# Tanveer81/ReVisionLLM

Measured on AMD Instinct MI355X. Metric: video-segments/sec (whole node), stage-2 100-seg recursion, Vicuna-7B, higher is better.
Workload: dtype fp16

## Files before the change

revisionllm_amd/build.py:

```python
import os
import subprocess
import sys
from concurrent.futures import ThreadPoolExecutor

HERE = os.path.dirname(os.path.abspath(__file__))
CSRC = os.path.join(HERE, "csrc")
OBJ = os.path.join(CSRC, "build")
FLAVOURS = {"f16": ("librevision_hip.so", "-DRV_OP_F16=1"), "bf16": ("librevision_hip_bf16.so", "-DRV_OP_F16=0")}
LIB = os.path.join(HERE, FLAVOURS["f16"][0])


def lib_path(flavour):
    return os.path.join(HERE, FLAVOURS[flavour][0])
SOURCES = ["error.hip", "init.hip", "gemm.hip", "gemm_pp.hip", "gemm_arows.hip", "gemm_rows.hip", "gemm_rows_p1.hip", "gemm_rows_p2.hip", "gemm_rows_p3.hip", "rowops.hip", "attention.hip", "sample.hip", "similarity.hip", "propose.hip", "prefilter.hip", "frames.hip", "frames_yuv.hip", "engine.hip"]
HEADERS = ["exports.map", "common.h", "kernels.h", "gemv_finish.h", "frames_common.h", "gemm_rows.hip", os.path.join("..", "..", "include", "revision_hip.h")]
FLAGS = ["--offload-arch=gfx950", "-O3", "-std=c++17", "-fPIC", "-fvisibility=hidden", "-fvisibility-inlines-hidden", "-Wall", "-Wno-unused-function",
         "-Wno-pass-failed"]


def _hipcc():
    for c in (os.environ.get("HIPCC"), "/opt/rocm/bin/hipcc", "hipcc"):
        if c and (os.path.isabs(c) and os.path.exists(c) or not os.path.isabs(c)):
            return c
    raise RuntimeError("hipcc not found")


def _stale(target, deps):
    if not os.path.exists(target):
        return True
    t = os.path.getmtime(target)
    return any(os.path.getmtime(d) > t for d in deps)


def build_library(force=False, verbose=False, flavours=("f16", "bf16")):
    hipcc = _hipcc()
    hdrs = [os.path.join(CSRC, h) for h in HEADERS]
    jobs = []
    for fl in flavours:
        os.makedirs(os.path.join(OBJ, fl), exist_ok=True)
        for s in SOURCES:
            src = os.path.join(CSRC, s)
            obj = os.path.join(OBJ, fl, s.replace(".hip", ".o"))
            if force or _stale(obj, [src] + hdrs):
                jobs.append([hipcc] + FLAGS + [FLAVOURS[fl][1], "-DRV_TU=" + s.replace(".hip", ""), "-c", src, "-o", obj])

    def run(cmd):
        r = subprocess.run(cmd, capture_output=True, text=True)
        if r.returncode != 0:
            raise RuntimeError("hipcc failed: %s\n%s" % (" ".join(cmd), r.stderr))
        if verbose and r.stderr:
            sys.stderr.write(r.stderr)

    with ThreadPoolExecutor(max_workers=int(os.environ.get("REVISION_BUILD_JOBS", "7"))) as ex:
        list(ex.map(run, jobs))
    for fl in flavours:
        objs = [os.path.join(OBJ, fl, s.replace(".hip", ".o")) for s in SOURCES]
        lib = lib_path(fl)
        if force or _stale(lib, objs):
            run([hipcc, "--offload-arch=gfx950", "-shared", "-fPIC", "-Wl,--version-script=" + os.path.join(CSRC, "exports.map"), "-o", lib] + objs)
    return LIB


if __name__ == "__main__":
    fl = tuple(a for a in sys.argv[1:] if a in FLAVOURS) or tuple(FLAVOURS)
    print(build_library(force="--force" in sys.argv, verbose=True, flavours=fl))
```

revisionllm_amd/csrc/gemm_rows.hip:

```cpp
#include <hip/hip_runtime.h>

#include <atomic>
#include <type_traits>

#include "kernels.h"
#include "gemv_finish.h"

#ifndef RS_PROBE
#define RS_PROBE 0
#endif
#ifndef RS_PART
#define RS_PART 0
#endif
#ifndef RS_DW_BIG
#define RS_DW_BIG 4
#endif

namespace {

typedef const __attribute__((address_space(1))) void* gptr_t;
typedef __attribute__((address_space(3))) void* lptr_t;
__device__ __forceinline__ void glds16(const void* g, void* l) { __builtin_amdgcn_global_load_lds((gptr_t)g, (lptr_t)l, 16, 0, 0); }

typedef unsigned int rs_u32x4 __attribute__((ext_vector_type(4)));
constexpr int RS_SC1 = 16;
__device__ __forceinline__ void st_sc1(__amdgpu_buffer_rsrc_t r, unsigned byte_off, f32x4 v) {
    __builtin_amdgcn_raw_buffer_store_b128(__builtin_bit_cast(rs_u32x4, v), r, (int)byte_off, 0, RS_SC1);
}
__device__ __forceinline__ f32x4 ld_sc1(__amdgpu_buffer_rsrc_t r, unsigned byte_off) {
    return __builtin_bit_cast(f32x4, __builtin_amdgcn_raw_buffer_load_b128(r, (int)byte_off, 0, RS_SC1));
}

constexpr int RS_W = 4;
constexpr int RS_THREADS = (RS_W + 1) * 64;
template <int MB, int WP = 1> struct RowsCfg {
    static constexpr int DW = WP == 2 ? 8 : (MB >= 8 ? RS_DW_BIG : 4), LPS = WP == 2 ? 2 : 4, DX = MB == 4 ? 4 : 3, WPE = MB <= 5 ? 3 : 2;
};
typedef unsigned int rs_w8 __attribute__((ext_vector_type(4)));

constexpr bool rows_sumsq_at_head(int MB) { return MB >= 8; }
template <int MB, int NTH, int PTB>
__device__ __forceinline__ void rows_sumsq(const GemvNorm& nrm, float* ssq, int tg) {
    if (!nrm.in_sumsq || (RS_PROBE & 16)) return;
    constexpr int CHAINS = MB * 128;
    constexpr int PT = (CHAINS + NTH - 1) / NTH;
    const int nblk = nrm.in_nblk;
    const int off = (RS_PROBE & 2048) ? 0 : (int)((blockIdx.x >> 3) * 37u) % CHAINS;
#pragma unroll
    for (int i0 = 0; i0 < PT; i0 += PTB) {
        f32x4 pj[PTB][8];
        int cc[PTB];
#pragma unroll
        for (int i = 0; i < PTB; ++i) {
            const int idx = tg + (i0 + i) * NTH;
            int c = idx + off;
            c = c >= CHAINS ? c - CHAINS : c;
            cc[i] = (i0 + i < PT && idx < CHAINS) ? c : -1;
            const int mb = c >> 7, q = (c >> 2) & 31, rq = c & 3;
            const float* src = nrm.in_sumsq + ((int64_t)(mb * nblk + q) * 16 + rq * 4);
#pragma unroll
            for (int j = 0; j < 8; ++j) {
                const bool have = q + 32 * j < nblk;
                const f32x4 v = *(const f32x4*)(src + (have ? j * 512 : 0));
                pj[i][j] = have ? v : f32x4{0.f, 0.f, 0.f, 0.f};
            }
        }
        __builtin_amdgcn_sched_barrier(0);
#pragma unroll
        for (int i = 0; i < PTB; ++i) {
            if (cc[i] < 0) continue;
            const int c = cc[i], mb = c >> 7, q = (c >> 2) & 31, rq = c & 3;
            f32x4 a = f32x4{0.f, 0.f, 0.f, 0.f};
#pragma unroll
            for (int j = 0; j < 8; ++j) a += pj[i][j];
            for (int b = q + 256; b < nblk; b += 32) a += *(const f32x4*)(nrm.in_sumsq + ((int64_t)(mb * nblk + b) * 16 + rq * 4));
            *(f32x4*)(ssq + mb * 512 + q * 16 + rq * 4) = a;
        }
    }
}

template <int MB>
__device__ __forceinline__ void rows_sumsq_total(const float* ssq, float* totl, int t) {
    if (t < MB * 16) {
        const int mb = t >> 4, row = t & 15;
        float tot = 0.f;
#pragma unroll
        for (int q = 0; q < 32; ++q) tot += ssq[(mb * 32 + q) * 16 + row];
        totl[t] = tot;
    }
}

template <int MB, int PPW, int PAIRS, int WP>
__device__ __forceinline__ void rows_qkv_finish(const f32x4 (&sres)[PPW], int wave, int cg, int fr, int kg, int M, const GemvNorm& nrm, const QkvRope& qr,
                                                const float* totl) {
    const int D = qr.H * 128;
    const int n0 = cg * 64;
    const int sec = n0 >= 2 * D ? 2 : n0 >= D ? 1 : 0;
    const int hd0 = n0 - sec * D, head = hd0 >> 7;
    int posv[PPW];
    f32x4 cf[PPW], wsc[PPW];
#pragma unroll
    for (int i = 0; i < PPW; ++i) {
        const int p = wave + RS_W * i < PAIRS ? wave + RS_W * i : PAIRS - 1;
        const int tile = p / MB, mb = p % MB, b = mb * 16 + fr;
        const int pc = (hd0 & 127) + tile * 16 + kg * 4;
        const int bc = b < M ? b : M - 1;
        posv[i] = b < M ? qr.row_pos[bc] : -1;
        cf[i] = sec < 2 ? *(const f32x4*)(qr.cs + ((int64_t)bc * 64 + (pc >> 1)) * 2) : f32x4{0.f, 0.f, 0.f, 0.f};
        if constexpr (WP == 2) wsc[i] = *(const f32x4*)(nrm.w_scale + n0 + tile * 16 + kg * 4);
    }
    __builtin_amdgcn_sched_barrier(0);
#pragma unroll
    for (int i = 0; i < PPW; ++i) {
        const int p = wave + RS_W * i;
        if (p >= PAIRS) break;
        const int tile = p / MB, mb = p % MB, b = mb * 16 + fr;
        const int pc = (hd0 & 127) + tile * 16 + kg * 4;
        f32x4 v = sres[i];
        if constexpr (WP == 2) v *= wsc[i];
        if (nrm.in_sumsq) v *= rsqrtf(__fmaf_rn(totl[mb * 16 + fr], nrm.inv_d, nrm.eps));
        const int pos = posv[i];
        if (pos < 0 || pos >= qr.Smax) continue;
        if (sec < 2) {
            const f32x4 t = cf[i];
            const float a0 = __fmaf_rn(v[0], t[0], -__fmul_rn(v[1], t[1])), b0 = __fmaf_rn(v[1], t[0], __fmul_rn(v[0], t[1]));
            const float a1 = __fmaf_rn(v[2], t[2], -__fmul_rn(v[3], t[3])), b1 = __fmaf_rn(v[3], t[2], __fmul_rn(v[2], t[3]));
            const u32x2 o = pack_op16x4(f32x4{a0, b0, a1, b1});
            if (sec == 0) *(u32x2*)((op16_t*)qr.q16 + (int64_t)b * D + hd0 + tile * 16 + kg * 4) = o;
            else *(u32x2*)((op16_t*)qr.kc + (((int64_t)b * qr.H + head) * qr.Smax + pos) * 128 + pc) = o;
        } else {
            op16_t* dst = (op16_t*)qr.vtc + ((int64_t)b * qr.H + head) * 128 * qr.Smax + rv_vt_index(pc, pos);
#pragma unroll
            for (int r = 0; r < 4; ++r) dst[r * 8] = f32_to_op16(v[r]);
        }
    }
}

#ifndef RS_PF_N
#define RS_PF_N 8
#endif
constexpr int RS_PF = RS_PF_N;
#ifndef RS_EARLY_READS
#define RS_EARLY_READS 0
#endif
constexpr bool rows_early(int MB) { return RS_EARLY_READS && MB >= 8 && !(RS_PROBE & (4 | 4096)); }
template <int MB, int WP>
__device__ __forceinline__ void rows_stage_schedule() {
#ifndef RS_NO_STAGE_SCHEDULE
    if constexpr (MB >= 8 && !(RS_PROBE & 4)) {
        constexpr int R = 4 * MB;
        if constexpr (!rows_early(MB)) __builtin_amdgcn_sched_group_barrier(0x100, RS_PF, 0);
#ifdef RS_EARLY_PIN_VMEM
        else __builtin_amdgcn_sched_group_barrier(0x020, WP == 2 ? 2 : 4, 0);
#endif
#pragma unroll
        for (int i = 0; i < R - RS_PF; ++i) {
            __builtin_amdgcn_sched_group_barrier(0x008, 1, 0);
            __builtin_amdgcn_sched_group_barrier(0x100, 1, 0);
        }
        __builtin_amdgcn_sched_group_barrier(0x008, RS_PF, 0);
    }
#endif
}

template <int MB, int VPW, int FIN, int WP = 1>
__global__ __attribute__((amdgpu_flat_work_group_size(RS_THREADS, RS_THREADS), amdgpu_waves_per_eu(RowsCfg<MB>::WPE, RowsCfg<MB>::WPE))) void
rows_kernel(const op16_t* __restrict__ X, const op16_t* __restrict__ W, float* __restrict__ planes, const float* __restrict__ bias,
            const float* res, int64_t ldr, void* Cv, int64_t ldc, int M, int N, int K, GemvNorm nrm, QkvRope qr) {
    extern __shared__ __attribute__((aligned(16))) char rs_smem[];
    constexpr int S = 8 / VPW, LOG = VPW == 8 ? 3 : VPW == 4 ? 2 : VPW == 2 ? 1 : 0;
    constexpr int DW = RowsCfg<MB, WP>::DW, DX = RowsCfg<MB, WP>::DX, LPS = RowsCfg<MB, WP>::LPS;
    constexpr int SLAB = MB * 4096;
    constexpr int XL = MB * 4;
    static_assert((DX - 2) * XL <= 63 && (DW - 2) * LPS <= 63, "vmcnt is a 6-bit counter");
    const int tid = threadIdx.x, lane = tid & 63;
    const int wave = __builtin_amdgcn_readfirstlane(tid >> 6);
    const int cg = blockIdx.x / S, sp = blockIdx.x % S;
    const int nkb = K >> 7;
    const int ntile = cg * RS_W + (wave < RS_W ? wave : 0);
    auto vcount = [&](int i) -> int { return (nkb - (sp * VPW + i) + 7) >> 3; };
    int T = 0;
#pragma unroll
    for (int i = 0; i < VPW; ++i) T += vcount(i);

    f32x4 acc[MB], stk[LOG ? LOG : 1][MB];
#pragma unroll
    for (int mb = 0; mb < MB; ++mb) acc[mb] = f32x4{0.f, 0.f, 0.f, 0.f};

    if (wave == RS_W) {
        int pi = 0, pc = 0;
        auto next_kb = [&]() -> int {
            int kb = -1;
            if (pi < VPW) {
                kb = sp * VPW + pi + 8 * pc;
                if (++pc == vcount(pi)) { pc = 0; ++pi; }
            }
            return kb;
        };
        auto issue = [&](int g) {
            const int kb = next_kb();
            const op16_t* xs = X + (kb >= 0 ? (int64_t)kb * (MB * 2048) : 0) + lane * 8;
            char* dst = rs_smem + (g % DX) * SLAB;
#pragma unroll
            for (int i = 0; i < XL; ++i) glds16(xs + i * 512, dst + i * 1024);
        };
        if constexpr (!(RS_PROBE & 8))
            for (int d = 0; d < DX - 1; ++d) issue(d);
        if constexpr (rows_sumsq_at_head(MB)) {
            if (nrm.in_sumsq && !(RS_PROBE & 16)) __builtin_amdgcn_s_barrier();
        }
        for (int g = 0; g < T; ++g) {
            asm volatile("s_waitcnt vmcnt(%0)" ::"n"((DX - 2) * XL) : "memory");
            if constexpr (!(RS_PROBE & 2)) __builtin_amdgcn_s_barrier();
            if constexpr (!(RS_PROBE & 8)) issue(g + DX - 1);
        }
        asm volatile("s_waitcnt vmcnt(0)" ::: "memory");
    } else {
        const op16_t* wp = W + (int64_t)ntile * (K >> 5) * (WP == 2 ? 256 : 512) + lane * 8;
        typename std::conditional<WP == 2, rs_w8, op16x8>::type wf[DW][LPS];
        int li = 0, lc = 0;
        int ci = 0, cc = 0;
#define RS_ISSUE_W(slot)                                                                                                             \
    do {                                                                                                                             \
        int kb_ = -1;                                                                                                                \
        if (li < VPW) {                                                                                                              \
            kb_ = sp * VPW + li + 8 * lc;                                                                                            \
            if (++lc == vcount(li)) { lc = 0; ++li; }                                                                                \
        }                                                                                                                            \
        const op16_t* ws_ = kb_ >= 0 ? ((RS_PROBE & 1) ? W + lane * 8 + (kb_ & 1) * 2048 : wp + (int64_t)((RS_PROBE & 8192) ? (kb_ + ((int)blockIdx.x * RS_W + wave) * 5) % nkb : kb_) * (WP == 2 ? 1024 : 2048)) : X + lane * 8; \
        _Pragma("unroll") for (int j_ = 0; j_ < LPS; ++j_)                                                                          \
            wf[slot][j_] = __builtin_nontemporal_load((const typename std::remove_reference<decltype(wf[0][0])>::type*)(ws_ + j_ * 512)); \
    } while (0)
#pragma unroll
        for (int d = 0; d < DW - 1; ++d) RS_ISSUE_W(d);
        if constexpr (rows_sumsq_at_head(MB)) {
            if (nrm.in_sumsq && !(RS_PROBE & 16)) {
                float* ssq_ = (float*)(rs_smem + DX * SLAB);
                rows_sumsq<MB, 256, 3>(nrm, ssq_, tid);
                asm volatile("s_waitcnt lgkmcnt(0)" ::: "memory");
                __builtin_amdgcn_s_barrier();
                rows_sumsq_total<MB>(ssq_, ssq_ + MB * 512, tid);
                asm volatile("s_waitcnt lgkmcnt(0)" ::: "memory");
            }
        }
        unsigned long long* stamps = (unsigned long long*)(rs_smem + DX * SLAB + MB * (2048 + 64));
        const bool stamping = (RS_PROBE & 16384) && S == 1 && wave == 0 && blockIdx.x == 8;
#define RS_STAMP(k_)                                                                       \
    if constexpr (RS_PROBE & 16384) {                                                      \
        if (stamping && g < 64) {                                                          \
            const unsigned long long t_ = __builtin_amdgcn_s_memtime();                    \
            if (lane == 0) stamps[g * 4 + (k_)] = t_;                                      \
        }                                                                                  \
    }
        if constexpr (RS_PROBE & 16384) {
            if (stamping) {
                for (int i = lane; i < 256; i += 64) stamps[i] = 0ull;
            }
        }
        for (int g0 = 0; g0 < T; g0 += DW) {
#pragma unroll
            for (int u = 0; u < DW; ++u) {
                const int g = g0 + u;
                if (g < T) {
                    RS_STAMP(0)
                    asm volatile("s_waitcnt vmcnt(%0)" ::"n"((DW - 2) * LPS) : "memory");
                    RS_STAMP(1)
                    if constexpr (!(RS_PROBE & 2)) __builtin_amdgcn_s_barrier();
                    RS_STAMP(2)
                    op16x8 pre[rows_early(MB) ? RS_PF : 1];
                    if constexpr (rows_early(MB)) {
                        const char* xs0 = rs_smem + (g % DX) * SLAB + lane * 16;
#pragma unroll
                        for (int i = 0; i < RS_PF; ++i) pre[i] = *(const op16x8*)(xs0 + i * 1024);
                    }
                    RS_ISSUE_W((u + DW - 1) % DW);
                    {
                        const char* xs = rs_smem + (g % DX) * SLAB + lane * 16;
#pragma unroll
                        for (int j = 0; j < 4; ++j) {
                            op16x8 wj;
                            if constexpr (WP == 2) wj = fp8x8_to_op16x8(wf[u][j >> 1][(j & 1) * 2], wf[u][j >> 1][(j & 1) * 2 + 1]);
                            else wj = wf[u][j];
#pragma unroll
                            for (int mb = 0; mb < MB; ++mb) {
                                const op16x8 xf = (rows_early(MB) && j * MB + mb < RS_PF) ? pre[(j * MB + mb) % RS_PF]
                                                                                           : *(const op16x8*)(xs + ((RS_PROBE & 4096) ? 0 : (j * MB + mb) * 1024));
                                if constexpr (RS_PROBE & 4) {
                                    if (mb == 0) acc[0][0] += __builtin_bit_cast(f32x4, wj)[j & 3] + __builtin_bit_cast(f32x4, xf)[0];
                                } else {
                                    acc[mb] = rv_mfma16(wj, xf, acc[mb]);
                                }
                            }
                        }
                        rows_stage_schedule<MB, WP>();
                    }
                    RS_STAMP(3)
                    if (++cc == vcount(ci)) {
                        if constexpr (VPW > 1) {
                            bool placed = false;
#pragma unroll
                            for (int b = 0; b < LOG; ++b) {
                                if (placed) continue;
                                if ((ci >> b) & 1) {
#pragma unroll
                                    for (int mb = 0; mb < MB; ++mb) acc[mb] = stk[b][mb] + acc[mb];
                                } else {
#pragma unroll
                                    for (int mb = 0; mb < MB; ++mb) stk[b][mb] = acc[mb];
                                    placed = true;
                                }
                            }
                            if (placed) {
#pragma unroll
                                for (int mb = 0; mb < MB; ++mb) acc[mb] = f32x4{0.f, 0.f, 0.f, 0.f};
                            }
                        }
                        cc = 0;
                        ++ci;
                    }
                }
            }
        }
#undef RS_ISSUE_W
#undef RS_STAMP
        if constexpr (RS_PROBE & 16384) {
            if (stamping) {
                asm volatile("s_waitcnt lgkmcnt(0)" ::: "memory");
                for (int i = lane; i < 256; i += 64) ((unsigned long long*)planes)[i] = stamps[i];
            }
        }
    }
    const unsigned plane = (unsigned)(N >> 4) * MB * 1024;
    const __amdgpu_buffer_rsrc_t pr = __builtin_amdgcn_make_buffer_rsrc(planes, 0, 0x7ffffff0, 0x00020000);
    constexpr int XCH_OFF = MB * 2048 > 16384 ? MB * 2048 : 16384;
    static_assert(XCH_OFF + RS_W * MB * 1024 <= DX * MB * 4096, "the exchange area must fit the slab ring");
    char* xch = rs_smem + XCH_OFF;
    if constexpr (S == 1) {
        asm volatile("s_waitcnt vmcnt(0)" ::: "memory");
        __syncthreads();
        if (wave < RS_W) {
#pragma unroll
            for (int mb = 0; mb < MB; ++mb) *(f32x4*)(xch + ((wave * MB + mb) * 64 + lane) * 16) = acc[mb];
        }
    } else {
        if (wave < RS_W) {
            const unsigned off = sp * plane + ((unsigned)ntile * MB * 64 + lane) * 16;
#pragma unroll
            for (int mb = 0; mb < MB; ++mb) st_sc1(pr, off + mb * 1024, acc[mb]);
        }
        asm volatile("s_waitcnt vmcnt(0)" ::: "memory");
    }
    __syncthreads();
    __shared__ int is_last;
    if constexpr (S > 1) {
        if (tid == 0) {
            unsigned* cnt = (unsigned*)nrm.arrive + (LOG * (RV_ROWS_COUNTERS / 4) + cg);
            is_last = __hip_atomic_fetch_add(cnt, 1u, __ATOMIC_RELAXED, __HIP_MEMORY_SCOPE_AGENT) % S == S - 1;
        }
        __syncthreads();
        if (!is_last) return;
    }
    constexpr int NT = (FIN == 1 || FIN == 2) ? 2 : 1;
    constexpr int OUT_BF16 = (FIN == 1 || FIN == 4) ? 1 : 0;
    constexpr int ACT = FIN == 1 ? RV_ACT_SILU_MUL : RV_ACT_NONE;
    constexpr int ROPE = FIN == 3 ? 1 : 0;
    constexpr int BPG = RS_W / NT;
    constexpr int PAIRS = BPG * MB;
    constexpr int PPW = (PAIRS + RS_W - 1) / RS_W;
    const int fr = lane & 15, kg = lane >> 4;
    const int nblk = N / (16 * NT);
    f32x4 pl[PPW][NT][S];
    if (wave < RS_W) {
#pragma unroll
        for (int i = 0; i < PPW; ++i) {
            const int p = wave + RS_W * i < PAIRS ? wave + RS_W * i : PAIRS - 1;
            const int blk = cg * BPG + p / MB, mb = p % MB;
#pragma unroll
            for (int t = 0; t < NT; ++t) {
                if constexpr (S == 1) {
                    pl[i][t][0] = *(const f32x4*)(xch + (((p / MB * NT + t) * MB + mb) * 64 + lane) * 16);
                } else {
                    const unsigned q = (((unsigned)(blk * NT + t) * MB + mb) * 64 + lane) * 16;
#pragma unroll
                    for (int w = 0; w < S; ++w) pl[i][t][w] = ld_sc1(pr, q + w * plane);
                }
            }
        }
    }
    float* ssq = (float*)(rs_smem + (rows_sumsq_at_head(MB) ? DX * SLAB : 0));
    if constexpr (!rows_sumsq_at_head(MB)) {
        if (nrm.in_sumsq && !(RS_PROBE & 16)) {
            rows_sumsq<MB, RS_THREADS, 2>(nrm, ssq, tid);
            __syncthreads();
            rows_sumsq_total<MB>(ssq, ssq + MB * 512, tid);
            __syncthreads();
        }
    }
    const float* totl = ssq + MB * 512;
    if (wave >= RS_W) return;
    if constexpr (ROPE) {
        if (qr.row_pos && qr.G == 1 && !(RS_PROBE & 64)) {
            f32x4 sv[PPW];
#pragma unroll
            for (int i = 0; i < PPW; ++i) {
                if constexpr (S == 8) sv[i] = gemv_tree8(pl[i][0]);
                else if constexpr (S == 4) sv[i] = (pl[i][0][0] + pl[i][0][1]) + (pl[i][0][2] + pl[i][0][3]);
                else if constexpr (S == 2) sv[i] = pl[i][0][0] + pl[i][0][1];
                else sv[i] = pl[i][0][0];
            }
            rows_qkv_finish<MB, PPW, PAIRS, WP>(sv, wave, cg, fr, kg, M, nrm, qr, totl);
            return;
        }
    }
#pragma unroll
    for (int i = 0; i < PPW; ++i) {
        const int p = wave + RS_W * i;
        if (p >= PAIRS) break;
        const int blk = cg * BPG + p / MB, mb = p % MB;
        f32x4 sres[NT];
#pragma unroll
        for (int t = 0; t < NT; ++t) {
            if constexpr (S == 8) sres[t] = gemv_tree8(pl[i][t]);
            else if constexpr (S == 4) sres[t] = (pl[i][t][0] + pl[i][t][1]) + (pl[i][t][2] + pl[i][t][3]);
            else if constexpr (S == 2) sres[t] = pl[i][t][0] + pl[i][t][1];
            else sres[t] = pl[i][t][0];
        }
        const float tot = nrm.in_sumsq ? totl[mb * 16 + fr] : 0.f;
        const f32x4 z = f32x4{0.f, 0.f, 0.f, 0.f};
        gemv_finish<NT, OUT_BF16, ACT, WP, ROPE>(sres, mb, fr, kg, blk, nblk, M, N, bias, res, ldr, Cv, ldc, nrm, qr, tot, z, z, z, z, false);
    }
}

constexpr int RS_MAXIT = 8;
template <int MB, int VPW, int FIN, int WP = 1>
__global__ __attribute__((amdgpu_flat_work_group_size(RS_THREADS, RS_THREADS), amdgpu_waves_per_eu(RowsCfg<MB>::WPE, RowsCfg<MB>::WPE))) void
rows_kernel_p(const op16_t* __restrict__ X, const op16_t* __restrict__ W, float* __restrict__ planes, const float* __restrict__ bias,
            const float* res, int64_t ldr, void* Cv, int64_t ldc, int M, int N, int K, GemvNorm nrm, QkvRope qr) {
    extern __shared__ __attribute__((aligned(16))) char rs_smem[];
    constexpr int S = 8 / VPW, LOG = VPW == 8 ? 3 : VPW == 4 ? 2 : VPW == 2 ? 1 : 0;
    constexpr int DW = RowsCfg<MB, WP>::DW, DX = RowsCfg<MB, WP>::DX, LPS = RowsCfg<MB, WP>::LPS;
    constexpr int SLAB = MB * 4096;
    constexpr int XL = MB * 4;
    static_assert((DX - 2) * XL <= 63 && (DW - 2) * LPS <= 63, "vmcnt is a 6-bit counter");
    const int tid = threadIdx.x, lane = tid & 63;
    const int wave = __builtin_amdgcn_readfirstlane(tid >> 6);
    const int nitems = (N >> 6) * S, G = (int)gridDim.x;
    const int sp = blockIdx.x % S;
    const int nkb = K >> 7;
    const int n_it = (nitems - (int)blockIdx.x + G - 1) / G;
    auto vcount = [&](int i) -> int { return (nkb - (sp * VPW + i) + 7) >> 3; };
    int T = 0;
#pragma unroll
    for (int i = 0; i < VPW; ++i) T += vcount(i);
    const int Tp = (T + DW - 1) / DW * DW;
    const unsigned plane = (unsigned)(N >> 4) * MB * 1024;
    const __amdgpu_buffer_rsrc_t pr = __builtin_amdgcn_make_buffer_rsrc(planes, 0, 0x7ffffff0, 0x00020000);

    f32x4 acc[MB], stk[LOG ? LOG : 1][MB];
#pragma unroll
    for (int mb = 0; mb < MB; ++mb) acc[mb] = f32x4{0.f, 0.f, 0.f, 0.f};

    if (wave == RS_W) {
        int pi = 0, pc = 0, pp = 0, pn = 0;
        auto issue = [&](int g) {
            int kb = -1;
            if (pn < n_it) {
                if (pp < T) {
                    kb = sp * VPW + pi + 8 * pc;
                    if (++pc == vcount(pi)) { pc = 0; ++pi; }
                }
                if (++pp == Tp) { pp = 0; pi = 0; ++pn; }
            }
            const op16_t* xs = X + (kb >= 0 ? (int64_t)kb * (MB * 2048) : 0) + lane * 8;
            char* dst = rs_smem + (g % DX) * SLAB;
#pragma unroll
            for (int i = 0; i < XL; ++i) glds16(xs + i * 512, dst + i * 1024);
        };
        if constexpr (!(RS_PROBE & 8))
            for (int d = 0; d < DX - 1; ++d) issue(d);
        if constexpr (rows_sumsq_at_head(MB)) {
            if (nrm.in_sumsq && !(RS_PROBE & 16)) __builtin_amdgcn_s_barrier();
        }
        const int TT = n_it * Tp;
        for (int g = 0; g < TT; ++g) {
            asm volatile("s_waitcnt vmcnt(%0)" ::"n"((DX - 2) * XL) : "memory");
            if constexpr (!(RS_PROBE & 2)) __builtin_amdgcn_s_barrier();
            if constexpr (!(RS_PROBE & 8)) issue(g + DX - 1);
        }
    } else {
        const int64_t tile_stride = (int64_t)(K >> 5) * (WP == 2 ? 256 : 512);
        const int64_t item_stride = (int64_t)(G / S) * RS_W * tile_stride;
        const op16_t* wp = W + ((int)blockIdx.x / S * RS_W + wave) * tile_stride + lane * 8;
        typename std::conditional<WP == 2, rs_w8, op16x8>::type wf[DW][LPS];
        int li = 0, lc = 0, lp = 0, ln = 0;
#define RS_ISSUE_W(slot)                                                                                                             \
    do {                                                                                                                             \
        const op16_t* ws_ = X + lane * 8;                                                                                            \
        if (ln < n_it) {                                                                                                             \
            if (lp < T) {                                                                                                            \
                const int kb_ = sp * VPW + li + 8 * lc;                                                                              \
                ws_ = (RS_PROBE & 1) ? W + lane * 8 + (kb_ & 1) * 2048 : wp + (int64_t)((RS_PROBE & 8192) ? (kb_ + ((int)blockIdx.x * RS_W + wave) * 5) % (K >> 7) : kb_) * (WP == 2 ? 1024 : 2048);                 \
                if (++lc == vcount(li)) { lc = 0; ++li; }                                                                            \
            }                                                                                                                        \
            if (++lp == Tp) { lp = 0; li = 0; ++ln; wp += item_stride; }                                                             \
        }                                                                                                                            \
        _Pragma("unroll") for (int j_ = 0; j_ < LPS; ++j_)                                                                          \
            wf[slot][j_] = __builtin_nontemporal_load((const typename std::remove_reference<decltype(wf[0][0])>::type*)(ws_ + j_ * 512)); \
    } while (0)
#pragma unroll
        for (int d = 0; d < DW - 1; ++d) RS_ISSUE_W(d);
        if constexpr (rows_sumsq_at_head(MB)) {
            if (nrm.in_sumsq && !(RS_PROBE & 16)) {
                float* ssq_ = (float*)(rs_smem + DX * SLAB);
                rows_sumsq<MB, 256, 3>(nrm, ssq_, tid);
                asm volatile("s_waitcnt lgkmcnt(0)" ::: "memory");
                __builtin_amdgcn_s_barrier();
                rows_sumsq_total<MB>(ssq_, ssq_ + MB * 512, tid);
                asm volatile("s_waitcnt lgkmcnt(0)" ::: "memory");
            }
        }
        int g = 0;
        for (int n = 0; n < n_it; ++n) {
            int ci = 0, cc = 0;
            for (int s0 = 0; s0 < Tp; s0 += DW) {
#pragma unroll
                for (int u = 0; u < DW; ++u, ++g) {
                    asm volatile("s_waitcnt vmcnt(%0)" ::"n"((DW - 2) * LPS) : "memory");
                    if constexpr (!(RS_PROBE & 2)) __builtin_amdgcn_s_barrier();
                    op16x8 pre[rows_early(MB) ? RS_PF : 1];
                    if constexpr (rows_early(MB)) {
                        const char* xs0 = rs_smem + (g % DX) * SLAB + lane * 16;
#pragma unroll
                        for (int i = 0; i < RS_PF; ++i) pre[i] = *(const op16x8*)(xs0 + i * 1024);
                    }
                    RS_ISSUE_W((u + DW - 1) % DW);
                    if (s0 + u < T) {
                        const char* xs = rs_smem + (g % DX) * SLAB + lane * 16;
#pragma unroll
                        for (int j = 0; j < 4; ++j) {
                            op16x8 wj;
                            if constexpr (WP == 2) wj = fp8x8_to_op16x8(wf[u][j >> 1][(j & 1) * 2], wf[u][j >> 1][(j & 1) * 2 + 1]);
                            else wj = wf[u][j];
#pragma unroll
                            for (int mb = 0; mb < MB; ++mb) {
                                const op16x8 xf = (rows_early(MB) && j * MB + mb < RS_PF) ? pre[(j * MB + mb) % RS_PF]
                                                                                           : *(const op16x8*)(xs + ((RS_PROBE & 4096) ? 0 : (j * MB + mb) * 1024));
                                if constexpr (RS_PROBE & 4) {
                                    if (mb == 0) acc[0][0] += __builtin_bit_cast(f32x4, wj)[j & 3] + __builtin_bit_cast(f32x4, xf)[0];
                                } else {
                                    acc[mb] = rv_mfma16(wj, xf, acc[mb]);
                                }
                            }
                        }
                        rows_stage_schedule<MB, WP>();
                        if (++cc == vcount(ci)) {
                            if constexpr (VPW > 1) {
                                bool placed = false;
#pragma unroll
                                for (int b = 0; b < LOG; ++b) {
                                    if (placed) continue;
                                    if ((ci >> b) & 1) {
#pragma unroll
                                        for (int mb = 0; mb < MB; ++mb) acc[mb] = stk[b][mb] + acc[mb];
                                    } else {
#pragma unroll
                                        for (int mb = 0; mb < MB; ++mb) stk[b][mb] = acc[mb];
                                        placed = true;
                                    }
                                }
                                if (placed) {
#pragma unroll
                                    for (int mb = 0; mb < MB; ++mb) acc[mb] = f32x4{0.f, 0.f, 0.f, 0.f};
                                }
                            }
                            cc = 0;
                            ++ci;
                        }
                    }
                }
            }
            if constexpr (S > 1) {
                const unsigned ntile = (unsigned)(((int)blockIdx.x + n * G) / S * RS_W + wave);
                const unsigned off = sp * plane + (ntile * MB * 64 + lane) * 16;
#pragma unroll
                for (int mb = 0; mb < MB; ++mb) {
                    st_sc1(pr, off + mb * 1024, acc[mb]);
                    acc[mb] = f32x4{0.f, 0.f, 0.f, 0.f};
                }
            }
        }
#undef RS_ISSUE_W
    }
    constexpr int XCH_OFF = MB * 2048 > 16384 ? MB * 2048 : 16384;
    static_assert(XCH_OFF + RS_W * MB * 1024 <= DX * MB * 4096, "the exchange area must fit the slab ring");
    char* xch = rs_smem + XCH_OFF;
    asm volatile("s_waitcnt vmcnt(0)" ::: "memory");
    __syncthreads();
    if constexpr (S == 1) {
        if (wave < RS_W) {
#pragma unroll
            for (int mb = 0; mb < MB; ++mb) *(f32x4*)(xch + ((wave * MB + mb) * 64 + lane) * 16) = acc[mb];
        }
        __syncthreads();
    }
    __shared__ int is_last[RS_MAXIT];
    if constexpr (S > 1) {
        if (tid < n_it) {
            unsigned* cnt = (unsigned*)nrm.arrive + (LOG * (RV_ROWS_COUNTERS / 4) + ((int)blockIdx.x + tid * G) / S);
            is_last[tid] = __hip_atomic_fetch_add(cnt, 1u, __ATOMIC_RELAXED, __HIP_MEMORY_SCOPE_AGENT) % S == S - 1;
        }
        __syncthreads();
        bool any = false;
        for (int n = 0; n < n_it; ++n) any = any || is_last[n];
        if (!any) return;
    }
    constexpr int NT = (FIN == 1 || FIN == 2) ? 2 : 1;
    constexpr int OUT_BF16 = (FIN == 1 || FIN == 4) ? 1 : 0;
    constexpr int ACT = FIN == 1 ? RV_ACT_SILU_MUL : RV_ACT_NONE;
    constexpr int ROPE = FIN == 3 ? 1 : 0;
    constexpr int BPG = RS_W / NT;
    constexpr int PAIRS = BPG * MB;
    constexpr int PPW = (PAIRS + RS_W - 1) / RS_W;
    const int fr = lane & 15, kg = lane >> 4;
    const int nblk = N / (16 * NT);
    float* ssq = (float*)(rs_smem + (rows_sumsq_at_head(MB) ? DX * SLAB : 0));
    if constexpr (!rows_sumsq_at_head(MB)) {
        if (nrm.in_sumsq && !(RS_PROBE & 16)) {
            rows_sumsq<MB, RS_THREADS, 2>(nrm, ssq, tid);
            __syncthreads();
            rows_sumsq_total<MB>(ssq, ssq + MB * 512, tid);
            __syncthreads();
        }
    }
    const float* totl = ssq + MB * 512;
    if (wave >= RS_W) return;
    for (int n = 0; n < n_it; ++n) {
        if constexpr (S > 1) {
            if (!is_last[n]) continue;
        }
        const int cg = ((int)blockIdx.x + n * G) / S;
        f32x4 pl[PPW][NT][S];
        if (wave < RS_W) {
#pragma unroll
            for (int i = 0; i < PPW; ++i) {
                const int p = wave + RS_W * i < PAIRS ? wave + RS_W * i : PAIRS - 1;
                const int blk = cg * BPG + p / MB, mb = p % MB;
#pragma unroll
                for (int t = 0; t < NT; ++t) {
                    if constexpr (S == 1) {
                        pl[i][t][0] = *(const f32x4*)(xch + (((p / MB * NT + t) * MB + mb) * 64 + lane) * 16);
                    } else {
                        const unsigned q = (((unsigned)(blk * NT + t) * MB + mb) * 64 + lane) * 16;
#pragma unroll
                        for (int w = 0; w < S; ++w) pl[i][t][w] = ld_sc1(pr, q + w * plane);
                    }
                }
            }
        }
#pragma unroll
        for (int i = 0; i < PPW; ++i) {
            const int p = wave + RS_W * i;
            if (p >= PAIRS) break;
            const int blk = cg * BPG + p / MB, mb = p % MB;
            f32x4 sres[NT];
#pragma unroll
            for (int t = 0; t < NT; ++t) {
                if constexpr (S == 8) sres[t] = gemv_tree8(pl[i][t]);
                else if constexpr (S == 4) sres[t] = (pl[i][t][0] + pl[i][t][1]) + (pl[i][t][2] + pl[i][t][3]);
                else if constexpr (S == 2) sres[t] = pl[i][t][0] + pl[i][t][1];
                else sres[t] = pl[i][t][0];
            }
            const float tot = nrm.in_sumsq ? totl[mb * 16 + fr] : 0.f;
            const f32x4 z = f32x4{0.f, 0.f, 0.f, 0.f};
            gemv_finish<NT, OUT_BF16, ACT, WP, ROPE>(sres, mb, fr, kg, blk, nblk, M, N, bias, res, ldr, Cv, ldc, nrm, qr, tot, z, z, z, z, false);
        }
    }
}

int rows_num_cus(int dev) {
    static std::atomic<int> cus[64];
    int n = cus[dev & 63].load(std::memory_order_relaxed);
    if (n == 0) {
        if (hipDeviceGetAttribute(&n, hipDeviceAttributeMultiprocessorCount, dev) != hipSuccess || n <= 0) n = 256;
        cus[dev & 63].store(n, std::memory_order_relaxed);
    }
    return n;
}
int rows_slots(int MBp) {
    int dev = 0;
    (void)hipGetDevice(&dev);
    return (rows_num_cus(dev) & ~7) * (MBp <= 5 ? 2 : 1);
}

int rows_splits(int64_t N, int MBp) {
    const int64_t cg = N / 64;
    int s = MBp >= 5 ? 2 : 1;
    const int fill = rv_cur_opts().rows_fill;
    if (MBp >= 8 && rv_cur_opts().rows_single && cg <= rows_slots(MBp) && cg * 4 >= (int64_t)rows_slots(MBp) * 3) return 1;
    while (s < 8 && cg * s < fill) s *= 2;
    if (rv_cur_opts().rows_persistent) {
        const int64_t slots = rows_slots(MBp);
        auto longest = [&](int s_) { return (cg * s_ + slots - 1) / slots * (8 / s_); };
        if (cg * s > slots)
            for (int s2 = s * 2; s2 <= 8; s2 *= 2)
                if (longest(s2) * 5 <= longest(s) * 4) s = s2;
    }
    return s;
}

#define RS_KERNEL (PERS ? rows_kernel_p<MB, VPW, FIN, WP> : rows_kernel<MB, VPW, FIN, WP>)
template <int MB, int VPW, int FIN, int WP, int PERS>
int rows_launch(const op16_t* X, const op16_t* W, const float* bias, const float* res, int64_t ldr, void* C, int64_t ldc, int M, int N, int K,
                const GemvNorm& nrm, const QkvRope& qr, hipStream_t st) {
    size_t lds = (size_t)RowsCfg<MB, WP>::DX * MB * 4096 + (rows_sumsq_at_head(MB) ? (size_t)MB * (2048 + 64) : 0)
                 + ((RS_PROBE & 16384) ? 2048 : 0);
    const unsigned items = (unsigned)(N / 64 * (8 / VPW));
    unsigned grid = items;
    if constexpr (PERS) {
        const unsigned slots = (unsigned)rows_slots(MB);
        if (slots >= 8 && slots < items) grid = slots;
    }
    RV_CHECK_ARG(items <= (unsigned)RS_MAXIT * grid, "gemm_rows: %u items for %u workgroups", items, grid);
    constexpr size_t alone = 81 * 1024;
    const bool spread = MB <= 5 && (int)grid <= rv_cur_opts().rows_spread;
    if (spread && lds < alone) lds = alone;
    static std::atomic<uint64_t> opted{0};
    int dev = 0;
    (void)hipGetDevice(&dev);
    const uint64_t bit = 1ull << (dev & 63);
    if (lds > 65536 && !(opted.load(std::memory_order_relaxed) & bit)) {
        if (hipFuncSetAttribute((const void*)RS_KERNEL, hipFuncAttributeMaxDynamicSharedMemorySize,
                                (int)(MB <= 5 && lds < alone ? alone : lds)) != hipSuccess) {
            rv_set_error("gemm_rows: cannot reserve %zu bytes of LDS", lds);
            return RV_ERR_HIP;
        }
        opted.fetch_or(bit, std::memory_order_relaxed);
    }
    hipLaunchKernelGGL((RS_KERNEL), dim3(grid), dim3(RS_THREADS), lds, st, X, W, nrm.planes, bias, res, ldr, C,
                       ldc, M, N, K, nrm, qr);
    return RV_OK;
}
#undef RS_KERNEL
template <int MB, int FIN, int WP>
int rows_by_split(int S, const op16_t* X, const op16_t* W, const float* bias, const float* res, int64_t ldr, void* C, int64_t ldc, int M, int N, int K,
                  const GemvNorm& nrm, const QkvRope& qr, hipStream_t st) {
    const bool pers = S > 1 && rv_cur_opts().rows_persistent && (int64_t)(N / 64) * S > rows_slots(MB) && (MB != 5 || S == 4);
#define RS_LAUNCH(VPW_) (pers ? rows_launch<MB, VPW_, FIN, WP, 1>(X, W, bias, res, ldr, C, ldc, M, N, K, nrm, qr, st) \
                              : rows_launch<MB, VPW_, FIN, WP, 0>(X, W, bias, res, ldr, C, ldc, M, N, K, nrm, qr, st))
    switch (S) {
        case 1: return rows_launch<MB, 8, FIN, WP, 0>(X, W, bias, res, ldr, C, ldc, M, N, K, nrm, qr, st);
        case 2: return RS_LAUNCH(4);
        case 4: return RS_LAUNCH(2);
        default: return RS_LAUNCH(1);
    }
#undef RS_LAUNCH
}
template <int FIN, int WP>
int rows_by_mb(int MBp, int S, const op16_t* X, const op16_t* W, const float* bias, const float* res, int64_t ldr, void* C, int64_t ldc, int M, int N,
               int K, const GemvNorm& nrm, const QkvRope& qr, hipStream_t st) {
#if RS_PART & 2
    return MBp == 8 ? rows_by_split<8, FIN, WP>(S, X, W, bias, res, ldr, C, ldc, M, N, K, nrm, qr, st)
                    : rows_by_split<9, FIN, WP>(S, X, W, bias, res, ldr, C, ldc, M, N, K, nrm, qr, st);
#else
    return MBp == 4 ? rows_by_split<4, FIN, WP>(S, X, W, bias, res, ldr, C, ldc, M, N, K, nrm, qr, st)
                    : rows_by_split<5, FIN, WP>(S, X, W, bias, res, ldr, C, ldc, M, N, K, nrm, qr, st);
#endif
}
template <int WP>
int rows_by_fin(int MBp, int S, const op16_t* X, const op16_t* W, const float* bias, const float* res, int64_t ldr, void* C, int64_t ldc, int out_dtype,
                int act, int M, int N, int K, const GemvNorm& nrm, const QkvRope* qr, hipStream_t st) {
    const QkvRope q0{};
    if (qr) return rows_by_mb<3, WP>(MBp, S, X, W, nullptr, nullptr, 0, nullptr, 0, M, N, K, nrm, *qr, st);
    if (act == RV_ACT_SILU_MUL) return rows_by_mb<1, WP>(MBp, S, X, W, bias, res, ldr, C, ldc, M, N, K, nrm, q0, st);
    if (N >= 16384 && out_dtype == RV_F32) return rows_by_mb<2, WP>(MBp, S, X, W, bias, res, ldr, C, ldc, M, N, K, nrm, q0, st);
    if (N < 16384 && out_dtype == RV_OP16) return rows_by_mb<4, WP>(MBp, S, X, W, bias, res, ldr, C, ldc, M, N, K, nrm, q0, st);
    if (N < 16384) return rows_by_mb<0, WP>(MBp, S, X, W, bias, res, ldr, C, ldc, M, N, K, nrm, q0, st);
    rv_set_error("gemm_rows: bf16 output with N >= 16384 is not instantiated");
    return RV_ERR_ARG;
}

}

#define RS_PART_FN_(n) gemm_rows_part##n
#define RS_PART_FN(n) RS_PART_FN_(n)
int RS_PART_FN(RS_PART)(int MBp, int S, const op16_t* X, const op16_t* W, const float* bias, const float* res, int64_t ldr, void* C, int64_t ldc,
                        int out_dtype, int act, int M, int N, int K, const GemvNorm& nrm, const QkvRope* qr, hipStream_t st) {
    return rows_by_fin<(RS_PART & 1) ? 2 : 1>(MBp, S, X, W, bias, res, ldr, C, ldc, out_dtype, act, M, N, K, nrm, qr, st);
}

#if RS_PART == 0
#define RS_PART_DECL(n)                                                                                                                      \
    int gemm_rows_part##n(int MBp, int S, const op16_t* X, const op16_t* W, const float* bias, const float* res, int64_t ldr, void* C, int64_t ldc, \
                          int out_dtype, int act, int M, int N, int K, const GemvNorm& nrm, const QkvRope* qr, hipStream_t st)
RS_PART_DECL(1);
RS_PART_DECL(2);
RS_PART_DECL(3);

size_t gemm_rows_ws_bytes() { return (size_t)(2 * 32768 / 16) * RV_XP_MAX_BLOCKS * 1024; }
extern "C" size_t rv_gemm_rows_ws_bytes(void) { return gemm_rows_ws_bytes(); }

int gemm_rows(const op16_t* X, const op16_t* W, const float* bias, const float* res, int64_t ldr, void* C, int64_t ldc, int out_dtype, int act,
              int M, int N, int K, hipStream_t st, const GemvNorm& nrm, const QkvRope* qr, int w_layout) {
    RV_CHECK_ARG(w_layout == 1 || (w_layout == 2 && nrm.w_scale), "gemm_rows: bf16 (1) or fp8 + per-row scales (2) fragment-packed weights");
    RV_CHECK_ARG(M > 32 && M <= RV_ROWS_MAX && nrm.x_packed == rv_xp_blocks(M) && nrm.planes && nrm.arrive,
                 "gemm_rows: 33 .. 144 fragment-packed rows, a plane workspace and arrival counters");
    RV_CHECK_ARG(N / 64 <= RV_ROWS_COUNTERS / 4, "gemm_rows: too many column groups");
    RV_CHECK_ARG(N % 64 == 0 && K % 128 == 0 && K >= 1024 && N <= 32768, "gemm_rows: N %% 64, K %% 128, K >= 1024, N <= 32768");
    RV_CHECK_ARG(act == RV_ACT_NONE || act == RV_ACT_SILU_MUL, "gemm_rows: no activation or SILU_MUL");
    RV_CHECK_ARG(act != RV_ACT_SILU_MUL || out_dtype == RV_OP16, "gemm_rows: SILU_MUL writes bf16");
    const int MBp = nrm.x_packed, S = rows_splits(N, MBp);
    RV_CHECK_ARG((size_t)S * (N / 16) * MBp * 1024 <= gemm_rows_ws_bytes(), "gemm_rows: %d partial planes of N = %d do not fit the plane workspace", S, N);
    auto* part = MBp >= 8 ? (w_layout == 2 ? gemm_rows_part3 : gemm_rows_part2) : (w_layout == 2 ? gemm_rows_part1 : gemm_rows_part0);
    const int rc = part(MBp, S, X, W, bias, res, ldr, C, ldc, out_dtype, act, M, N, K, nrm, qr, st);
    if (rc) return rc;
    RV_CHECK_LAUNCH("gemm_rows");
    return RV_OK;
}

extern "C" int rv_gemm_rows(const void* Xp, const void* Wp, const float* w_scale, void* C, int32_t M, int32_t N, int32_t K, void* planes,
                            int32_t* arrive, int act, int out_dtype, void* stream) {
    RV_CHECK_ARG(Xp && Wp && C && planes && arrive, "rv_gemm_rows: null argument");
    GemvNorm nrm;
    nrm.w_scale = w_scale;
    nrm.x_packed = rv_xp_blocks(M);
    nrm.planes = (float*)planes;
    nrm.arrive = arrive;
    const int ldc = act == RV_ACT_SILU_MUL ? N / 2 : N;
    return gemm_rows((const op16_t*)Xp, (const op16_t*)Wp, nullptr, nullptr, 0, C, ldc, out_dtype, act, M, N, K, (hipStream_t)stream, nrm, nullptr,
                     w_scale ? 2 : 1);
}
#endif
```

Measured before the change: 6501.

## Add two-tile-per-wave rows GEMM kernel for wide N with MB>=8

Adds a new rows_kernel_w where each wave computes two 16-column tiles, so every X fragment staged in LDS is reused across two weight tiles. Weights are prefetched into registers several stages deep with nontemporal loads, and the MFMA, LDS-read and global-load interleaving is pinned with sched_group_barrier hints. Partial sums are folded through a register and LDS stack instead of a split-K plane workspace. It is used for bf16 weights with N >= 16384 and 8 or more packed row blocks (MB 9 only for the gated SiLU case), which targets the MLP up/gate projection. The aim is less X re-reading and no split-K reduction traffic, at the cost of fewer workgroups, one wave per EU, and a larger LDS footprint.

Result: no change. 6513, median of 5 (+0.2%).

```diff
diff --git a/revisionllm_amd/build.py b/revisionllm_amd/build.py
--- a/revisionllm_amd/build.py
+++ b/revisionllm_amd/build.py
@@ -12,7 +12,7 @@
 
 def lib_path(flavour):
     return os.path.join(HERE, FLAVOURS[flavour][0])
-SOURCES = ["error.hip", "init.hip", "gemm.hip", "gemm_pp.hip", "gemm_arows.hip", "gemm_rows.hip", "gemm_rows_p1.hip", "gemm_rows_p2.hip", "gemm_rows_p3.hip", "rowops.hip", "attention.hip", "sample.hip", "similarity.hip", "propose.hip", "prefilter.hip", "frames.hip", "frames_yuv.hip", "engine.hip"]
+SOURCES = ["error.hip", "init.hip", "gemm.hip", "gemm_pp.hip", "gemm_arows.hip", "gemm_rows.hip", "gemm_rows_p1.hip", "gemm_rows_p2.hip", "gemm_rows_p3.hip", "gemm_rows_p4.hip", "rowops.hip", "attention.hip", "sample.hip", "similarity.hip", "propose.hip", "prefilter.hip", "frames.hip", "frames_yuv.hip", "engine.hip"]
 HEADERS = ["exports.map", "common.h", "kernels.h", "gemv_finish.h", "frames_common.h", "gemm_rows.hip", os.path.join("..", "..", "include", "revision_hip.h")]
 FLAGS = ["--offload-arch=gfx950", "-O3", "-std=c++17", "-fPIC", "-fvisibility=hidden", "-fvisibility-inlines-hidden", "-Wall", "-Wno-unused-function",
          "-Wno-pass-failed"]
diff --git a/revisionllm_amd/csrc/gemm_rows.hip b/revisionllm_amd/csrc/gemm_rows.hip
--- a/revisionllm_amd/csrc/gemm_rows.hip
+++ b/revisionllm_amd/csrc/gemm_rows.hip
@@ -677,6 +677,208 @@
     }
 }
 
+constexpr int RW_DW = 4;
+template <int MB, int PF>
+__device__ __forceinline__ void rows_w_stage_schedule() {
+    constexpr int R = 4 * MB;
+    __builtin_amdgcn_sched_group_barrier(0x020, 8, 0);
+    __builtin_amdgcn_sched_group_barrier(0x100, PF, 0);
+#pragma unroll
+    for (int i = 0; i < R - PF; ++i) {
+        __builtin_amdgcn_sched_group_barrier(0x008, 2, 0);
+        __builtin_amdgcn_sched_group_barrier(0x100, 1, 0);
+    }
+    __builtin_amdgcn_sched_group_barrier(0x008, 2 * PF, 0);
+}
+template <int MB>
+__device__ __forceinline__ void rows_w_tail_schedule() {
+    __builtin_amdgcn_sched_group_barrier(0x200, MB, 0);
+    __builtin_amdgcn_sched_group_barrier(0x020, MB, 0);
+}
+
+template <int MB, int FIN>
+__global__ __attribute__((amdgpu_flat_work_group_size(256, 256), amdgpu_waves_per_eu(1, 1))) void
+rows_kernel_w(const op16_t* __restrict__ X, const op16_t* __restrict__ W, const float* __restrict__ bias,
+              const float* res, int64_t ldr, void* Cv, int64_t ldc, int M, int N, int K, GemvNorm nrm, QkvRope qr) {
+    extern __shared__ __attribute__((aligned(16))) char rs_smem[];
+    constexpr int VPW = 8;
+    constexpr int DW = RW_DW, WP = 1, PF = RS_PF;
+    constexpr int SLAB = MB * 4096;
+    const int tid = threadIdx.x, lane = tid & 63;
+    const int wave = __builtin_amdgcn_readfirstlane(tid >> 6);
+    const int cg = blockIdx.x;
+    const int nkb = K >> 7;
+    const int ntile = cg * 8 + wave * 2;
+    auto vcount = [&](int i) -> int { return (nkb - i + 7) >> 3; };
+
+    f32x4 acc[2][MB], stk0[2][MB], stk1[2][MB];
+#pragma unroll
+    for (int t = 0; t < 2; ++t)
+#pragma unroll
+        for (int mb = 0; mb < MB; ++mb) acc[t][mb] = f32x4{0.f, 0.f, 0.f, 0.f};
+
+    const int64_t tile_stride = (int64_t)(K >> 5) * 512;
+    const op16_t* wp = W + (int64_t)ntile * tile_stride + lane * 8;
+    op16x8 wf[DW][2][4], xr[MB];
+    int li = 0, lc = 0;
+    int xi = 0, xc = 0;
+    auto next_kb = [&](int& vi, int& vc) -> int {
+        int kb = -1;
+        if (vi < VPW) {
+            const int n = vcount(vi), np = vi < VPW - 1 ? (n + DW - 1) / DW * DW : n;
+            if (vc < n) kb = vi + 8 * vc;
+            if (++vc == np) { vc = 0; ++vi; }
+        }
+        return kb;
+    };
+    const op16_t *ws_, *xs_;
+    int64_t t1_;
+#define RW_NEXT_W()                                                                                                           \
+    do {                                                                                                                      \
+        const int kb_ = next_kb(li, lc);                                                                                      \
+        ws_ = kb_ >= 0 ? wp + (int64_t)kb_ * 2048 : X + lane * 8;                                   \
+        t1_ = kb_ >= 0 ? tile_stride : 0;                                                                                     \
+    } while (0)
+#define RW_ISSUE_W(slot)                                                                                                      \
+    do {                                                                                                                      \
+        _Pragma("unroll") for (int j_ = 0; j_ < 4; ++j_) {                                                                    \
+            wf[slot][0][j_] = __builtin_nontemporal_load((const op16x8*)(ws_ + j_ * 512));                                    \
+            wf[slot][1][j_] = __builtin_nontemporal_load((const op16x8*)(ws_ + t1_ + j_ * 512));                              \
+        }                                                                                                                     \
+    } while (0)
+#define RW_NEXT_X()                                                                                                           \
+    do {                                                                                                                      \
+        const int kb_ = next_kb(xi, xc);                                                                                      \
+        xs_ = X + (kb_ >= 0 ? (int64_t)kb_ * (MB * 2048) + wave * (MB * 512) : 0) + lane * 8;                                 \
+    } while (0)
+#define RW_ISSUE_X()                                                                                                          \
+    do {                                                                                                                      \
+        _Pragma("unroll") for (int i_ = 0; i_ < MB; ++i_) xr[i_] = *(const op16x8*)(xs_ + i_ * 512);                         \
+    } while (0)
+#define RW_WRITE_X(slot)                                                                                                      \
+    do {                                                                                                                      \
+        char* xd_ = rs_smem + (slot) * SLAB + wave * (MB * 1024) + lane * 16;                                                 \
+        _Pragma("unroll") for (int i_ = 0; i_ < MB; ++i_) *(op16x8*)(xd_ + i_ * 1024) = xr[i_];                              \
+    } while (0)
+
+    RW_NEXT_X();
+    RW_ISSUE_X();
+#pragma unroll
+    for (int d = 0; d < DW - 1; ++d) {
+        RW_NEXT_W();
+        RW_ISSUE_W(d);
+    }
+    char* const park = rs_smem + 2 * SLAB;
+    float* const totl = (float*)(rs_smem + 4 * SLAB);
+    if (nrm.in_sumsq) {
+        rows_sumsq<MB, 256, 3>(nrm, (float*)park, tid);
+        asm volatile("s_waitcnt lgkmcnt(0)" ::: "memory");
+        __builtin_amdgcn_s_barrier();
+        rows_sumsq_total<MB>((const float*)park, totl, tid);
+    }
+    RW_WRITE_X(0);
+    RW_NEXT_X();
+    RW_ISSUE_X();
+#pragma unroll
+    for (int i = 0; i < VPW; ++i) {
+        const int cnt = vcount(i), np = i < VPW - 1 ? (cnt + DW - 1) / DW * DW : cnt;
+        for (int s0 = 0; s0 < np; s0 += DW) {
+#pragma unroll
+            for (int u = 0; u < DW; ++u) {
+                if (s0 + u < np) {
+                    RW_NEXT_W();
+                    RW_NEXT_X();
+                    asm volatile("s_waitcnt lgkmcnt(0)" ::: "memory");
+                    __builtin_amdgcn_s_barrier();
+                    RW_ISSUE_W((u + DW - 1) % DW);
+                    if (s0 + u < cnt) {
+                        const char* xs = rs_smem + (u & 1) * SLAB + lane * 16;
+                        op16x8 xq[PF];
+#pragma unroll
+                        for (int r = 0; r < PF; ++r) xq[r] = *(const op16x8*)(xs + r * 1024);
+#pragma unroll
+                        for (int r = 0; r < 4 * MB; ++r) {
+                            const op16x8 xf = xq[r % PF];
+                            acc[0][r % MB] = rv_mfma16(wf[u][0][r / MB], xf, acc[0][r % MB]);
+                            acc[1][r % MB] = rv_mfma16(wf[u][1][r / MB], xf, acc[1][r % MB]);
+                            if (r + PF < 4 * MB) xq[r % PF] = *(const op16x8*)(xs + (r + PF) * 1024);
+                        }
+                        rows_w_stage_schedule<MB, PF>();
+                    }
+                    RW_WRITE_X((u + 1) & 1);
+                    RW_ISSUE_X();
+                    rows_w_tail_schedule<MB>();
+                }
+            }
+        }
+#define RW_FOLD_ADD(STK) \
+    _Pragma("unroll") for (int t = 0; t < 2; ++t) _Pragma("unroll") for (int mb = 0; mb < MB; ++mb) { acc[t][mb] = STK[t][mb] + acc[t][mb]; __builtin_amdgcn_sched_barrier(0); }
+#define RW_FOLD_PUSH(STK) \
+    _Pragma("unroll") for (int t = 0; t < 2; ++t) _Pragma("unroll") for (int mb = 0; mb < MB; ++mb) { STK[t][mb] = acc[t][mb]; acc[t][mb] = f32x4{0.f, 0.f, 0.f, 0.f}; }
+        if (!(i & 1)) {
+            RW_FOLD_PUSH(stk0);
+        } else {
+            RW_FOLD_ADD(stk0);
+            if (!(i & 2)) {
+                RW_FOLD_PUSH(stk1);
+            } else {
+                RW_FOLD_ADD(stk1);
+#pragma unroll
+                for (int t = 0; t < 2; ++t)
+#pragma unroll
+                    for (int mb = 0; mb < MB; ++mb) {
+                        f32x4* pk = (f32x4*)(park + (((wave * 2 + t) * MB + mb) * 64 + lane) * 16);
+                        if (!(i & 4)) {
+                            *pk = acc[t][mb];
+                            acc[t][mb] = f32x4{0.f, 0.f, 0.f, 0.f};
+                        } else {
+                            acc[t][mb] = *pk + acc[t][mb];
+                        }
+                        __builtin_amdgcn_sched_barrier(0);
+                    }
+            }
+        }
+#undef RW_FOLD_ADD
+#undef RW_FOLD_PUSH
+    }
+#undef RW_NEXT_W
+#undef RW_NEXT_X
+#undef RW_ISSUE_W
+#undef RW_ISSUE_X
+#undef RW_WRITE_X
+    static_assert(DW % 2 == 0, "the slab slot of a stage is taken from the unroll index");
+    char* xch = rs_smem;
+    asm volatile("s_waitcnt vmcnt(0) lgkmcnt(0)" ::: "memory");
+    __syncthreads();
+#pragma unroll
+    for (int t = 0; t < 2; ++t)
+#pragma unroll
+        for (int mb = 0; mb < MB; ++mb) *(f32x4*)(xch + (((wave * 2 + t) * MB + mb) * 64 + lane) * 16) = acc[t][mb];
+    __syncthreads();
+    constexpr int NT = (FIN == 1 || FIN == 2) ? 2 : 1;
+    constexpr int OUT_BF16 = (FIN == 1 || FIN == 4) ? 1 : 0;
+    constexpr int ACT = FIN == 1 ? RV_ACT_SILU_MUL : RV_ACT_NONE;
+    constexpr int BPG = RS_W / NT;
+    constexpr int PAIRS = BPG * MB;
+    constexpr int PPW = (PAIRS + RS_W - 1) / RS_W;
+    const int fr = lane & 15, kg = lane >> 4;
+    const int nblk = N / (16 * NT);
+    for (int half = 0; half < 2; ++half) {
+#pragma unroll
+        for (int i = 0; i < PPW; ++i) {
+            const int p = wave + RS_W * i;
+            if (p >= PAIRS) break;
+            const int blk = (cg * 2 + half) * BPG + p / MB, mb = p % MB;
+            f32x4 sres[NT];
+#pragma unroll
+            for (int t = 0; t < NT; ++t) sres[t] = *(const f32x4*)(xch + (((half * RS_W + p / MB * NT + t) * MB + mb) * 64 + lane) * 16);
+            const float tot = nrm.in_sumsq ? totl[mb * 16 + fr] : 0.f;
+            const f32x4 z = f32x4{0.f, 0.f, 0.f, 0.f};
+            gemv_finish<NT, OUT_BF16, ACT, WP, 0>(sres, mb, fr, kg, blk, nblk, M, N, bias, res, ldr, Cv, ldc, nrm, qr, tot, z, z, z, z, false);
+        }
+    }
+}
+
 int rows_num_cus(int dev) {
     static std::atomic<int> cus[64];
     int n = cus[dev & 63].load(std::memory_order_relaxed);
@@ -741,6 +943,32 @@
     return RV_OK;
 }
 #undef RS_KERNEL
+bool rows_wide(int64_t N, int MBp, int w_layout, bool gated) {
+    return MBp >= 8 && w_layout == 1 && N % 128 == 0 && N >= 16384 && N / 128 * 2 > rows_slots(MBp) && (MBp == 8 || gated);
+}
+template <int MB, int FIN>
+int rows_launch_w(const op16_t* X, const op16_t* W, const float* bias, const float* res, int64_t ldr, void* C, int64_t ldc, int M, int N, int K,
+                  const GemvNorm& nrm, const QkvRope& qr, hipStream_t st) {
+    if constexpr ((FIN == 1 || FIN == 2) && (MB == 8 || FIN == 1)) {
+        const size_t lds = (size_t)4 * MB * 4096 + (size_t)MB * 64;
+        static std::atomic<uint64_t> opted{0};
+        int dev = 0;
+        (void)hipGetDevice(&dev);
+        const uint64_t bit = 1ull << (dev & 63);
+        if (!(opted.load(std::memory_order_relaxed) & bit)) {
+            if (hipFuncSetAttribute((const void*)rows_kernel_w<MB, FIN>, hipFuncAttributeMaxDynamicSharedMemorySize, (int)lds) != hipSuccess) {
+                rv_set_error("gemm_rows: cannot reserve %zu bytes of LDS", lds);
+                return RV_ERR_HIP;
+            }
+            opted.fetch_or(bit, std::memory_order_relaxed);
+        }
+        hipLaunchKernelGGL((rows_kernel_w<MB, FIN>), dim3((unsigned)(N / 128)), dim3(256), lds, st, X, W, bias, res, ldr, C, ldc, M, N, K, nrm, qr);
+        return RV_OK;
+    } else {
+        rv_set_error("gemm_rows: no two-tile kernel for this finish at %d row blocks", MB);
+        return RV_ERR_ARG;
+    }
+}
 template <int MB, int FIN, int WP>
 int rows_by_split(int S, const op16_t* X, const op16_t* W, const float* bias, const float* res, int64_t ldr, void* C, int64_t ldc, int M, int N, int K,
                   const GemvNorm& nrm, const QkvRope& qr, hipStream_t st) {
@@ -758,7 +986,10 @@
 template <int FIN, int WP>
 int rows_by_mb(int MBp, int S, const op16_t* X, const op16_t* W, const float* bias, const float* res, int64_t ldr, void* C, int64_t ldc, int M, int N,
                int K, const GemvNorm& nrm, const QkvRope& qr, hipStream_t st) {
-#if RS_PART & 2
+#if RS_PART == 4
+    return MBp == 8 ? rows_launch_w<8, FIN>(X, W, bias, res, ldr, C, ldc, M, N, K, nrm, qr, st)
+                    : rows_launch_w<9, FIN>(X, W, bias, res, ldr, C, ldc, M, N, K, nrm, qr, st);
+#elif RS_PART & 2
     return MBp == 8 ? rows_by_split<8, FIN, WP>(S, X, W, bias, res, ldr, C, ldc, M, N, K, nrm, qr, st)
                     : rows_by_split<9, FIN, WP>(S, X, W, bias, res, ldr, C, ldc, M, N, K, nrm, qr, st);
 #else
@@ -795,6 +1026,7 @@
 RS_PART_DECL(1);
 RS_PART_DECL(2);
 RS_PART_DECL(3);
+RS_PART_DECL(4);
 
 size_t gemm_rows_ws_bytes() { return (size_t)(2 * 32768 / 16) * RV_XP_MAX_BLOCKS * 1024; }
 extern "C" size_t rv_gemm_rows_ws_bytes(void) { return gemm_rows_ws_bytes(); }
@@ -808,9 +1040,11 @@
     RV_CHECK_ARG(N % 64 == 0 && K % 128 == 0 && K >= 1024 && N <= 32768, "gemm_rows: N %% 64, K %% 128, K >= 1024, N <= 32768");
     RV_CHECK_ARG(act == RV_ACT_NONE || act == RV_ACT_SILU_MUL, "gemm_rows: no activation or SILU_MUL");
     RV_CHECK_ARG(act != RV_ACT_SILU_MUL || out_dtype == RV_OP16, "gemm_rows: SILU_MUL writes bf16");
-    const int MBp = nrm.x_packed, S = rows_splits(N, MBp);
+    const int MBp = nrm.x_packed;
+    const bool wide = !qr && rows_wide(N, MBp, w_layout, act == RV_ACT_SILU_MUL);
+    const int S = wide ? 1 : rows_splits(N, MBp);
     RV_CHECK_ARG((size_t)S * (N / 16) * MBp * 1024 <= gemm_rows_ws_bytes(), "gemm_rows: %d partial planes of N = %d do not fit the plane workspace", S, N);
-    auto* part = MBp >= 8 ? (w_layout == 2 ? gemm_rows_part3 : gemm_rows_part2) : (w_layout == 2 ? gemm_rows_part1 : gemm_rows_part0);
+    auto* part = wide ? gemm_rows_part4 : MBp >= 8 ? (w_layout == 2 ? gemm_rows_part3 : gemm_rows_part2) : (w_layout == 2 ? gemm_rows_part1 : gemm_rows_part0);
     const int rc = part(MBp, S, X, W, bias, res, ldr, C, ldc, out_dtype, act, M, N, K, nrm, qr, st);
     if (rc) return rc;
     RV_CHECK_LAUNCH("gemm_rows");
diff --git a/revisionllm_amd/csrc/gemm_rows_p4.hip b/revisionllm_amd/csrc/gemm_rows_p4.hip
--- /dev/null
+++ b/revisionllm_amd/csrc/gemm_rows_p4.hip
@@ -0,0 +1,2 @@
+#define RS_PART 4
+#include "gemm_rows.hip"
```
